# jaeyoungjo99/ELiMaLoc

Measured on AMD Instinct MI355X. Metric: ICP registrations/sec, 128k-pt scan vs 10M-pt map; pose err vs CPU ref, higher is better.
Workload: dtype f64

## Files before the change

### elimaloc_amd/_lib.py

```python
import ctypes as C
import os

_HERE = os.path.dirname(os.path.abspath(__file__))
LIB_PATH = os.environ.get("ELM_LIB") or os.path.join(_HERE, "libelimaloc_hip.so")

ELM_OK = 0
P2P, GICP, VGICP, AVGICP = 0, 1, 2, 3
MAX_ITER_TRACE = 64
PACKED_SUMS = 32
COMM_ID_BYTES = 128


class ElmError(RuntimeError):
    pass


class RegConfig(C.Structure):
    _fields_ = [
        ("i_max_thread", C.c_int32),
        ("icp_method", C.c_int32),
        ("voxel_search_method", C.c_int32),
        ("use_radar_cov", C.c_int32),
        ("max_iteration", C.c_int32),
        ("b_debug_print", C.c_int32),
# ... 109 lines not shown
                ("max_score_points", C.c_int32), ("top_k", C.c_int32), ("nms_xy_m", C.c_double), ("nms_yaw_deg", C.c_double),
                ("pool_min", C.c_int32), ("max_kz_span", C.c_int32), ("bitmap_max_bytes", C.c_int64)]


class GlobalRelocStats(C.Structure):
    _fields_ = [("lattice_poses", C.c_int64), ("valid_leaves", C.c_int64), ("nx", C.c_int32), ("ny", C.c_int32), ("n_yaw", C.c_int32),
                ("levels", C.c_int32), ("n_counted", C.c_int32), ("passes", C.c_int32), ("tau", C.c_uint32), ("_pad", C.c_uint32),
                ("nodes_bounded", C.c_int64 * 24), ("nodes_kept", C.c_int64 * 24), ("leaves_scored", C.c_int64), ("point_evals", C.c_int64),
                ("ms_ground", C.c_double), ("ms_search", C.c_double), ("ms_refine", C.c_double)]


ALLREDUCE_FN = C.CFUNCTYPE(C.c_int, C.c_void_p, C.c_size_t, C.c_void_p, C.c_void_p)

EXPORTS = [
    "elm_reg_config_default", "elm_ctx_create", "elm_ctx_create_multi", "elm_ctx_group_info", "elm_register_shard", "elm_ctx_destroy", "elm_last_error", "elm_strerror",
    "elm_ctx_synchronize", "elm_ctx_stream", "elm_ctx_set_profiling", "elm_ctx_set_work_counters", "elm_ctx_get_profile", "elm_map_build", "elm_map_destroy", "elm_map_cal_voxel_cov_all",
    "elm_map_cal_point_cov_all", "elm_map_build_neighbourhoods", "elm_map_get_info", "elm_map_empty", "elm_map_download_points",
    "elm_map_download_voxels", "elm_map_find_ground_height", "elm_map_get_correspondences", "elm_align_clouds_local", "elm_scan_upload", "elm_scan_destroy",
    "elm_scan_size", "elm_scan_download", "elm_register", "elm_format_register_log", "elm_register_batch", "elm_register_stream", "elm_register_stream_host", "elm_host_alloc", "elm_host_free", "elm_ctx_measure_h2d", "elm_register_batch_enqueue",
    "elm_register_batch_finish", "elm_deskew", "elm_deskew_downsample", "elm_deskew_prepare", "elm_comm_get_unique_id", "elm_comm_init",
    "elm_comm_destroy", "elm_comm_info", "elm_comm_set_hook", "elm_filter_points_by_distance", "elm_voxel_downsample",
    "elm_get_interpolated_pose", "elm_shape_odom_covariance", "elm_cal_frame_point_cov",
    "elm_ekf_config_default", "elm_ekf_create", "elm_ekf_destroy", "elm_ekf_predict_imu", "elm_ekf_predict", "elm_ekf_update_can", "elm_gps_project", "elm_ekf_update_navsatfix",
    "elm_ekf_update_pose", "elm_ekf_update_pcm_odom", "elm_ekf_get_state", "elm_ekf_publish",
    "elm_ini_load", "elm_ini_destroy", "elm_ini_get_string", "elm_ini_get_int", "elm_ini_get_bool", "elm_ini_get_double",
    "elm_ini_get_array", "elm_pcm_node_config_default", "elm_load_pcm_config", "elm_load_ekf_config", "elm_pcd_load_xyz",
    "elm_free", "elm_scan_from_cloud", "elm_pcm_callback_point_cloud",
    "elm_reloc_config_default", "elm_reloc_make_hypotheses", "elm_map_score_poses", "elm_relocalize",
    "elm_reloc_global_config_default", "elm_map_ground_heights", "elm_reloc_global_hypotheses", "elm_relocalize_global",
]

# ... 63 lines not shown
    L.elm_ctx_group_info.argtypes = [vp, C.POINTER(C.c_int), C.POINTER(C.c_int), C.POINTER(C.c_int), C.c_int]
    L.elm_register_shard.argtypes = [vp, vp, fp, C.c_size_t, C.c_size_t, dp, C.POINTER(RegConfig), C.POINTER(RegResult), C.POINTER(IterTrace), C.c_int]
    L.elm_ctx_destroy.restype = None
    L.elm_last_error.argtypes = [vp]
    L.elm_last_error.restype = C.c_char_p
    L.elm_strerror.argtypes = [C.c_int]
    L.elm_strerror.restype = C.c_char_p
    L.elm_ctx_synchronize.argtypes = [vp]
    L.elm_ctx_stream.argtypes = [vp]
    L.elm_ctx_stream.restype = vp
    L.elm_format_register_log.argtypes = [C.POINTER(RegConfig), C.POINTER(RegResult), C.c_size_t, C.POINTER(IterTrace), C.POINTER(C.c_double),
                                          C.c_double, C.c_char_p, C.c_size_t]
    L.elm_format_register_log.restype = C.c_size_t
    L.elm_ctx_set_profiling.argtypes = [vp, C.c_int]
    L.elm_ctx_set_work_counters.argtypes = [vp, C.c_int]
    L.elm_ctx_get_profile.argtypes = [vp, C.POINTER(Profile), C.c_int]
    L.elm_map_build.argtypes = [vp, fp, C.c_size_t, C.c_double, C.c_int, C.POINTER(vp)]
    L.elm_map_destroy.argtypes = [vp]
    L.elm_map_destroy.restype = None
    L.elm_map_cal_voxel_cov_all.argtypes = [vp]
    L.elm_map_cal_point_cov_all.argtypes = [vp, C.c_double]
    L.elm_map_build_neighbourhoods.argtypes = [vp]
    L.elm_map_get_info.argtypes = [vp, C.POINTER(MapInfo)]
    L.elm_map_empty.argtypes = [vp]
    L.elm_map_download_points.argtypes = [vp, dp, dp, dp, C.c_size_t]
    L.elm_map_download_voxels.argtypes = [vp, C.POINTER(C.c_int32), C.POINTER(C.c_int32), dp, dp, C.c_size_t]
    L.elm_map_find_ground_height.argtypes = [vp, C.c_double, C.c_double, dp, ip]
    L.elm_cal_frame_point_cov.argtypes = [dp, C.c_size_t, C.c_double, C.c_double, C.c_double, dp]
    L.elm_align_clouds_local.argtypes = [vp, C.c_int, dp, dp, dp, dp, C.c_size_t, dp, C.c_double, C.POINTER(RegConfig), dp, dp, dp]
    L.elm_map_get_correspondences.argtypes = [vp, vp, C.c_int, dp, C.c_size_t, C.c_double, C.POINTER(C.c_uint32), C.POINTER(C.c_int32), C.c_size_t, C.POINTER(C.c_size_t)]
# ... 95 lines not shown
```

### elimaloc_amd/csrc/elm_api.cpp

```cpp
#include <dlfcn.h>
#include <hip/hip_runtime.h>
#include <math.h>
#include <stdio.h>
#include <stdlib.h>
#include <string.h>
#include <unistd.h>

#include <algorithm>
#include <chrono>
#include <map>
#include <mutex>
#include <new>
#include <set>
#include <string>
#include <thread>
#include <vector>

#include "elm_hostapi.hpp"
#include "elm_internal.hpp"
#include "elm_la.hpp"

using namespace elm;

struct DevBuf {
// ... 62 lines not shown
    int device = 0;
    uint64_t id = 0;
    hipStream_t stream = nullptr;
    hipStream_t copy_stream = nullptr, order_stream = nullptr, poll_stream = nullptr;
    hipEvent_t ev_iter[4] = {nullptr, nullptr, nullptr, nullptr};
    std::vector<hipEvent_t> ev_groups;
    uint16_t* d_hilbert = nullptr;
    DevBuf d_order_jobs, d_order_tmp, d_arena, d_raw, d_flagged, d_asym;
    DevBuf d_q0, d_q1, d_q2, d_q3, d_q4, d_q5;
    DevBuf d_reloc[16];
    bool work_counters = false;
    void* h_jobs = nullptr;
    size_t h_jobs_cap = 0;
    std::string last_error;
    DevBuf d_scans, d_state, d_partials, d_sums, d_T0, d_trace, d_stage_pts, d_active, d_queue, d_ds;
    int stream_hint_count = 0, stream_hint_slots = 0, stream_hint_iters = 0;
    int* h_active = nullptr;
    int iter_hint = 0;
    int iter_ring[8] = {0, 0, 0, 0, 0, 0, 0, 0};
    unsigned iter_ring_pos = 0;
    const void* iter_key_map = nullptr;
    int iter_key_method = -1, iter_key_batch = 0;
    void* h_state = nullptr;
    size_t h_state_cap = 0;
    void* h_trace = nullptr;
    size_t h_trace_cap = 0;
    void* h_stage = nullptr;
    size_t h_stage_cap = 0;
    std::vector<uint32_t> h_key, h_ord, h_tmp;
    std::vector<struct elm_scan*> scan_free;
// ... 170 lines not shown
    {
        std::lock_guard<std::mutex> lk(g_live_mu);
        if (!g_live_ctx.erase(ctx)) return;
    }
    (void)hipSetDevice(ctx->device);
    if (ctx->stream) (void)hipStreamSynchronize(ctx->stream);
    if (ctx->comm && g_rccl.comm_destroy) g_rccl.comm_destroy(ctx->comm);
    for (hipStream_t st : {ctx->copy_stream, ctx->order_stream, ctx->poll_stream})
        if (st) { (void)hipStreamSynchronize(st); (void)hipStreamDestroy(st); }
    for (hipEvent_t e : {ctx->ev_iter[0], ctx->ev_iter[1], ctx->ev_iter[2], ctx->ev_iter[3]})
        if (e) (void)hipEventDestroy(e);
    for (hipEvent_t e : ctx->ev_groups) (void)hipEventDestroy(e);
    if (ctx->d_hilbert) (void)hipFree(ctx->d_hilbert);
    if (ctx->h_jobs) (void)hipHostFree(ctx->h_jobs);
    DevBuf* bufs[] = {&ctx->d_scans, &ctx->d_state, &ctx->d_partials, &ctx->d_sums, &ctx->d_T0, &ctx->d_trace, &ctx->d_stage_pts, &ctx->d_active, &ctx->d_queue, &ctx->d_ds,
                      &ctx->d_order_jobs, &ctx->d_order_tmp, &ctx->d_arena, &ctx->d_raw, &ctx->d_flagged, &ctx->d_asym, &ctx->d_q0, &ctx->d_q1, &ctx->d_q2, &ctx->d_q3, &ctx->d_q4, &ctx->d_q5};
    if (ctx->h_active) (void)hipHostFree(ctx->h_active);
    for (DevBuf* b : bufs)
        if (b->p) (void)hipFree(b->p);
    for (DevBuf& b : ctx->d_reloc)
        if (b.p) (void)hipFree(b.p);
    for (auto& b : ctx->scan_pool) (void)hipFree(b.first);
    for (elm_scan* f : ctx->scan_free) delete f;
    if (ctx->h_state) (void)hipHostFree(ctx->h_state);
    if (ctx->h_trace) (void)hipHostFree(ctx->h_trace);
    if (ctx->h_stage) (void)hipHostFree(ctx->h_stage);
    if (ctx->h_desc) (void)hipHostFree(ctx->h_desc);
    for (hipEvent_t e : ctx->events) (void)hipEventDestroy(e);
    if (ctx->stream) (void)hipStreamDestroy(ctx->stream);
    delete ctx;
}

extern "C" const char* elm_last_error(const elm_ctx* ctx) { return ctx ? ctx->last_error.c_str() : ""; }
extern "C" void* elm_ctx_stream(elm_ctx* ctx) { return ctx ? (void*)ctx->stream : nullptr; }
extern "C" int elm_ctx_set_work_counters(elm_ctx* ctx, int enable) {
    if (!ctx) return ELM_ERR_INVALID;
    if (ctx->in_flight) return ELM_ERR_INVALID;
    if (group_call(ctx)) return elm_multi::set_work_counters(ctx, enable);
    ctx->work_counters = enable != 0;
    return ELM_OK;
}

extern "C" int elm_ctx_set_profiling(elm_ctx* ctx, int enable) {
    if (!ctx) return ELM_ERR_INVALID;
    ctx->profiling = enable != 0;
    return ELM_OK;
}
extern "C" int elm_ctx_get_profile(elm_ctx* ctx, elm_profile* out, int reset) {
    if (!ctx || !out) return ELM_ERR_INVALID;
// ... 1578 lines not shown
    rp.method = cfg->icp_method;
    rp.max_iter = cfg->max_iteration;
    rp.uniform_blocks = uniform_blocks;
    rp.radar = pc.radar ? (cfg->use_radar_cov != 0 ? 1 : 2) : 0;
    rp.stats = ctx->work_counters ? 1 : 0;
    rp.radar_var[0] = cfg->range_variance_m;
    rp.radar_var[1] = cfg->azimuth_variance_deg;
    rp.radar_var[2] = cfg->elevation_variance_deg;
    if (pc.asym) {
        int rc;
        if ((rc = dev_reserve(ctx, ctx->d_asym, (size_t)std::max<uint32_t>(blocks, 1) * kAsymRecord * sizeof(double))) != ELM_OK) return rc;
        rp.asym = (double*)ctx->d_asym.p;
        rp.asym_sums = (double*)ctx->d_sums.p + (size_t)n_scans * kSums;
    }
    rp.rank_check = ((ctx->comm || ctx->hook) && !rp.radar && !rp.stats) ? 1 : 0;
    ctx->rp = rp;
    return ELM_OK;
}

static bool reg_args_ok(const elm_ctx* ctx, const elm_map* map, const elm_reg_config* cfg) {
    return map->ctx == ctx && cfg->icp_method >= ELM_P2P && cfg->icp_method <= ELM_AVGICP && !ctx->in_flight;
}

struct StateTail {
    int32_t active;
    int32_t rank_mismatch;
    int32_t _pad0[2];
    uint32_t ds_kept;
    int32_t ds_overflow;
    int32_t _pad1[10];
// ... 1074 lines not shown
```

### elimaloc_amd/csrc/elm_internal.hpp

```cpp
#pragma once
#include <hip/hip_runtime.h>
#include <stdint.h>

#include "../../include/elimaloc_hip.h"

namespace elm {

struct __attribute__((aligned(32))) HashSlot {
    int32_t kx, ky, kz;
    int32_t vid;
    uint32_t start;
    uint32_t cnt;
    uint32_t pad0, pad1;
};

struct __attribute__((packed, aligned(4))) Pt3 {
    float x, y, z;
};

struct __attribute__((aligned(16))) GridBlk {
    float x[4], y[4], z[4];
};

struct __attribute__((aligned(64))) VoxRec {
// ... 84 lines not shown

struct ScanState {
    double T[16];
    double Rinv[9];
    double tinv[3];
    double fitness;
    double local_cov[36];
    double n_corr_last;
    double pt_iters, cand_total, occ_total, fallback_blocks, tested_total;
    int32_t done;
    int32_t success;
    int32_t gate;
    int32_t iters;
    int32_t reg;
    int32_t _pad;
};

struct QueueItem {
    const Pt3* pts;
    uint32_t n, n_total;
};
struct StreamCtrl {
    int32_t next;
    int32_t completed;
    int32_t total;
    int32_t ready;
    int32_t done_iter;
};

struct StreamArgs {
// ... 17 lines not shown
    double max_fitness;
    int32_t method;
    int32_t max_iter;
    uint32_t uniform_blocks;
    int32_t radar;
    int32_t _reserved0;
    int32_t stats;
    uint32_t* flagged;
    int32_t rank_check;
    int32_t _pad_rc;
    double* asym;
    double* asym_sums;
    double radar_var[3];
    const double* query;
    int32_t* q_out;
};
constexpr int kAsymRecord = 16;
constexpr int kRadarRecord = 64;

constexpr int kTileShift = 3, kTile = 1 << kTileShift;
constexpr int kBlock = 256;
constexpr int kInitPack = 8;
struct InitPack {
    ScanDesc d[kInitPack];
    double T0[kInitPack][16];
};
constexpr int kSums = ELM_PACKED_SUMS;

void launch_init_state(hipStream_t s, ScanState* st, const double* T0, int batch, int map_empty, int* active);
void launch_init_pack(hipStream_t s, ScanDesc* scans, ScanState* st, const InitPack& pack, int batch, int map_empty, int* active, const unsigned* n_dev);
void launch_stream_refill(hipStream_t s, ScanDesc* scans, ScanState* st, int slots, const QueueItem* queue, const double* qT0,
                          ScanState* out_state, StreamCtrl* ctrl, int first, int save = 1);
// ... 108 lines not shown
```

### elimaloc_amd/csrc/elm_k_grid.hip

```cpp
#include <float.h>
#include <algorithm>
#include <hip/hip_runtime.h>

#include "elm_internal.hpp"
#include "elm_la.hpp"
#include "elm_dev_grid.hpp"

namespace elm {

template <int METHOD, int COMPACT, int TILED, int STATS, int WIDE>
__global__ __launch_bounds__(kBlock, (METHOD == ELM_P2P ? (STATS ? 7 : kGridWaves) : kGicpWaves)) void k_accumulate_grid(
       const DevMap m, const ScanDesc* __restrict__ scans, int batch,
                                                                            unsigned total_blocks, const ScanState* __restrict__ st,
                                                                            double* __restrict__ partials, const RegParams rp) {
    constexpr int kStats = (STATS == 1) ? 1 : 0;
    constexpr bool QUERY = STATS == 2;
    constexpr int NV = (METHOD == ELM_P2P) ? (kStats ? kP2PVals : kP2PVals - 3) : kSums;
    __shared__ double s_buf[kRedPass * kBlock];
    __shared__ double s_red[kSums];
    __shared__ int s_res[kBlock];
    __shared__ int s_tst[kStats ? kBlock : 1];
    __shared__ float s_pz[METHOD == ELM_P2P ? kBlock : 1];
    __shared__ unsigned s_st[kStats ? kBlock : 1];
    __shared__ unsigned s_cnt[kBlock / 64];
// ... 21 lines not shown
        double* p = s_buf + threadIdx.x;
        p[4 * kBlock] = a; p[5 * kBlock] = b; p[6 * kBlock] = c; p[7 * kBlock] = d;
    };
    auto load_g = [&](double& gx, double& gy, double& gz, float& pxf, float& pyf) {
        const double* p = s_buf + threadIdx.x;
        gx = p[4 * kBlock]; gy = p[5 * kBlock]; gz = p[6 * kBlock];
        const double w = p[7 * kBlock];
        pxf = __int_as_float(__double2loint(w)); pyf = __int_as_float(__double2hiint(w));
    };
    auto transform = [&](const float4 pf, double& px, double& py, double& pz, double& gx, double& gy, double& gz) {
        px = pf.x; py = pf.y; pz = pf.z;
        gx = ((S.T[0] * px + S.T[4] * py) + S.T[8] * pz) + S.T[12];
        gy = ((S.T[1] * px + S.T[5] * py) + S.T[9] * pz) + S.T[13];
        gz = ((S.T[2] * px + S.T[6] * py) + S.T[10] * pz) + S.T[14];
    };
    if (valid) {
        double px, py, pz, gx, gy, gz;
        float4 pf = make_float4(0.f, 0.f, 0.f, 0.f);
        if (QUERY) {
            gx = rp.query[3 * (size_t)i]; gy = rp.query[3 * (size_t)i + 1]; gz = rp.query[3 * (size_t)i + 2];
            px = py = pz = 0.0;
        } else {
            const Pt3 p3 = sd.pts[i];
            pf = make_float4(p3.x, p3.y, p3.z, 0.f);
            transform(pf, px, py, pz, gx, gy, gz);
        }
        const GridAxis ax = grid_axis(gx, m), ay = grid_axis(gy, m), az = grid_axis(gz, m);
        unsigned stat = 0;
        if (kStats && !TILED) {
            const int ux = ax.f - m.vx0, uy = ay.f - m.vy0, uz = az.f - m.vz0;
            const bool in_box = (unsigned)ux < (unsigned)m.vnx && (unsigned)uy < (unsigned)m.vny && (unsigned)uz < (unsigned)m.vnz;
            const unsigned sidx = in_box ? ((unsigned)ux * (unsigned)m.vny + (unsigned)uy) * (unsigned)m.vnz + (unsigned)uz : 0u;
            stat = m.vox_stat[sidx];
            stat = in_box ? stat : 0u;
        }
        float rho_u = 3e38f;
        int bx0, bx1, by0, by1, bz0, bz1;
        int ox, oy, oz;
        float dxo, dyo, dzo;
        grid_lean(ax, bx0, bx1, rho_u, ox, dxo);
        grid_lean(ay, by0, by1, rho_u, oy, dyo);
        grid_lean(az, bz0, bz1, rho_u, oz, dzo);
        (void)oz; (void)dzo;
        const int rx0 = bx0 - m.gx0, rx1 = bx1 - m.gx0, ry0 = by0 - m.gy0, ry1 = by1 - m.gy0, rz0 = bz0 - m.gz0, rz1 = bz1 - m.gz0;
        const bool inside = rx0 >= 0 && rx1 < m.gnx && rx0 <= rx1 && ry0 >= 0 && ry1 < m.gny && ry0 <= ry1 && rz0 >= 0 && rz1 < m.gnz && rz0 <= rz1;
        unsigned sb[4];
        int cb[5];
        cb[0] = 0;
        const float ex_ = fmaxf(dxo * (float)h - 1e-6f, 0.f), ey_ = fmaxf(dyo * (float)h - 1e-6f, 0.f);
        const float Bx = fminf(ex_ * ex_, 1e36f), By = fminf(ey_ * ey_, 1e36f);
        const bool xfirst = Bx <= By, has_x = rx1 != rx0, has_y = ry1 != ry0;
        unsigned s0[4], s1[4], s2[4];
        bool ok[4];
        ok[0] = inside;
        ok[1] = inside && (xfirst ? has_x : has_y);
        ok[2] = inside && (xfirst ? has_y : has_x);
        ok[3] = inside && has_x && has_y;
        if (!TILED) {
            const int own_x = ox ? rx1 : rx0, own_y = oy ? ry1 : ry0;
            const unsigned base = ((unsigned)own_x * (unsigned)m.gny + (unsigned)own_y) * (unsigned)m.gnz + (unsigned)rz0;
            const unsigned xs = (unsigned)m.gny * (unsigned)m.gnz, ys = (unsigned)m.gnz;
            const unsigned cx_n = ox ? base - xs : base + xs, cy_n = oy ? base - ys : base + ys, cd = ox ? cy_n - xs : cy_n + xs;
            unsigned cellv[4];
            cellv[0] = base; cellv[1] = xfirst ? cx_n : cy_n; cellv[2] = xfirst ? cy_n : cx_n; cellv[3] = cd;
#pragma unroll
            for (int k = 0; k < 4; ++k) {
                const uint32_t* e = m.grid_start + (ok[k] ? cellv[k] : 0u);
                s0[k] = e[0]; s1[k] = e[1]; s2[k] = e[2];
            }
        } else {
            const int own_x = ox ? rx1 : rx0, oth_x = ox ? rx0 : rx1, own_y = oy ? ry1 : ry0, oth_y = oy ? ry0 : ry1;
            int cxv[4], cyv[4];
            cxv[0] = own_x; cyv[0] = own_y;
            cxv[1] = xfirst ? oth_x : own_x; cyv[1] = xfirst ? own_y : oth_y;
            cxv[2] = xfirst ? own_x : oth_x; cyv[2] = xfirst ? oth_y : own_y;
            cxv[3] = oth_x; cyv[3] = oth_y;
#pragma unroll
            for (int k = 0; k < 4; ++k) {
                int zc0, nzc;
                const uint32_t* e = col_cells<1>(m, ok[k] ? cxv[k] : 0, ok[k] ? cyv[k] : 0, rz0, rz1, zc0, nzc);
                s0[k] = e[0]; s1[k] = e[nzc]; s2[k] = s1[k];
            }
        }
        float rr = (rho_u < 1e30f) ? (rho_u * (float)h - 1.1e-6f) * 0.999998f : 1e18f;
        float rr2 = (rr > 0.f) ? rr * rr * 0.999999f : -1.f;
        float ghx = (float)gx, ghy = (float)gy, ghz = (float)gz;
        const float eg = (fabsf(ghx) + fabsf(ghy) + fabsf(ghz)) * 5.9604652e-08f;
        float egrr = (2.0f * eg * fmaxf(rr, 0.f) + eg * eg) * 1.000001f;
        float egblk = (7.0f * eg * (float)h + eg * eg) * 1.000001f;
        float L1 = fminf(Bx, By), L2 = fmaxf(Bx, By), L3 = (Bx + By) * 0.999999f;
        asm volatile("" : "+v"(rr2), "+v"(ghx), "+v"(ghy), "+v"(ghz), "+v"(egrr), "+v"(egblk), "+v"(L1), "+v"(L2), "+v"(L3));
        stash_w(gx, gy, gz, __hiloint2double(__float_as_int(pf.y), __float_as_int(pf.x)));
        if (METHOD == ELM_P2P) s_pz[threadIdx.x] = pf.z;
        if (kStats) s_st[threadIdx.x] = stat;
        {
            int b0v[4], b1v[4];
#pragma unroll
            for (int k = 0; k < 4; ++k) {
                b0v[k] = ok[k] ? (int)s0[k] : 0;
                b1v[k] = ok[k] ? (int)((rz1 > rz0 || TILED) ? s2[k] : s1[k]) : 0;
            }
#pragma unroll
            for (int k = 0; k < 4; ++k) {
                sb[k] = (unsigned)(b0v[k] - cb[k]) * kBlkStep;
                cb[k + 1] = cb[k] + (b1v[k] - b0v[k]);
            }
        }
        {
            int nblk = cb[4];
            const f32x2 gxy = {ghx, ghy}, gzz = {ghz, 0.f};
            unsigned m1 = 0x7F800000u, m2 = 0x7F800000u;
            unsigned jb = 0;
            for (int t0 = 0; t0 < nblk; t0 += kBlocksPerTrip) {
                unsigned pb[kBlocksPerTrip];
#pragma unroll
                for (int w = 0; w < kBlocksPerTrip; ++w) {
                    const int t = t0 + w;
                    unsigned b_ = sb[3];
#pragma unroll
                    for (int k = 2; k >= 0; --k) b_ = (t < cb[k + 1]) ? sb[k] : b_;
                    pb[w] = (t < nblk) ? b_ + (unsigned)t * kBlkStep : 0u;
                }
                GridBlk B[kBlocksPerTrip];
#pragma unroll
                for (int w = 0; w < kBlocksPerTrip; ++w)
                    B[w] = *reinterpret_cast<const GridBlk*>(reinterpret_cast<const char*>(lp) + (WIDE ? ((size_t)pb[w] << 4) : (size_t)pb[w]));
                __builtin_amdgcn_sched_barrier(0);
#pragma unroll
                for (int w = 0; w < kBlocksPerTrip; ++w) {
                    f32x2 da, db;
                    blk_dist_h(B[w], gxy, gzz, da, db);
                    const unsigned was = m1;
                    two_smallest(da.x, 0u, m1, m2);
                    two_smallest(da.y, 1u, m1, m2);
                    two_smallest(db.x, 2u, m1, m2);
                    two_smallest(db.y, 3u, m1, m2);
                    jb = (m1 != was) ? pb[w] : jb;
                }
                const float dbest = __uint_as_float(m1 & ~3u);
                const float best = (dbest < rr2) ? (dbest + dbest * 7.62939453125e-06f + 2.0f * egrr) * 1.000001f : __builtin_inff();
                nblk = (L1 > best) ? cb[1] : ((L2 > best) ? cb[2] : ((L3 > best) ? cb[3] : nblk));
            }
            n_tested = 4 * nblk;
            hard = true;
            if (jb > 0) {
                const float d1 = __uint_as_float(m1 & ~3u), d2 = __uint_as_float(m2 & ~3u);
                const float r2 = d1 + d1 * 3.814697265625e-06f + egrr;
                hr2 = d1 + d1 * 3.814697265625e-06f + egblk;
                if (d2 - d2 * 3.814697265625e-06f > r2 + egrr && r2 < rr2) {
                    bj = (int)(jb / kBlkStep) * 4 + (int)(m1 & 3u);
                    hard = false;
                }
            }
        }
    }
    const unsigned long long hm = __ballot(hard);
    const unsigned lane = threadIdx.x & 63u, wave = threadIdx.x >> 6;
    if (lane == 0) s_cnt[wave] = (unsigned)__popcll(hm);
    __syncthreads();
    unsigned n_hard = 0, my_slot = 0;
#pragma unroll
    for (unsigned w = 0; w < kBlock / 64; ++w) {
        my_slot += (w < wave) ? s_cnt[w] : 0u;
        n_hard += s_cnt[w];
    }
    my_slot += (unsigned)__popcll(hm & ((1ull << lane) - 1ull));
    if (n_hard) {
        GridHardRec* __restrict__ s_rec = reinterpret_cast<GridHardRec*>(s_buf);
        if (hard) {
// ... 13 lines not shown
            const GridHardRec R = s_rec[live ? it : 0];
            int win, walked;
            grid_ball_walk<TILED, LPI>(m, lp, R, live, rl, lane, win, walked);
            if (kStats) walked = group_sum_int<LPI>(walked);
            if (rl == 0 && live) {
                s_res[it] = win;
                if (kStats) s_tst[it] = walked;
            }
        }
        __syncthreads();
        if (hard) {
            bj = s_res[my_slot];
            if (kStats) n_tested += s_tst[my_slot];
        }
        __syncthreads();
    }
    if (QUERY) {
        if (valid) {
            double gx, gy, gz;
            float pxf, pyf;
            load_g(gx, gy, gz, pxf, pyf);
            int out = -2;
            if (bj >= 0) {
                const Pt3 q = blk_point(lp, bj);
                const double ex = (double)q.x - gx, ey = (double)q.y - gy, ez = (double)q.z - gz;
                if ((ex * ex + ey * ey) + ez * ez < rp.th2) out = (int)m.grid_idx[bj];
            } else if ((gx * gx + gy * gy) + gz * gz < rp.th2) {
                out = -1;
            }
            rp.q_out[i] = out;
// ... 127 lines not shown
```

### elimaloc_amd/csrc/elm_k_solve.hip

```cpp
#include <float.h>
#include <algorithm>
#include <hip/hip_runtime.h>

#include "elm_internal.hpp"
#include "elm_la.hpp"
#include "elm_dev_reduce.hpp"

namespace elm {

__device__ void update_inverse(ScanState& S) {
    double R[9];
    for (int r = 0; r < 3; ++r)
        for (int c = 0; c < 3; ++c) R[r * 3 + c] = S.T[c * 4 + r];
    inv3(R, S.Rinv);
    for (int r = 0; r < 3; ++r)
        S.tinv[r] = -((S.Rinv[r * 3] * S.T[12] + S.Rinv[r * 3 + 1] * S.T[13]) + S.Rinv[r * 3 + 2] * S.T[14]);
}

__device__ void init_scan_state(ScanState& S, const double* __restrict__ T0, int reg, int map_empty) {
    for (int k = 0; k < 16; ++k) S.T[k] = T0[k];
    update_inverse(S);
    S.fitness = 0.0;
    for (int k = 0; k < 36; ++k) S.local_cov[k] = (k % 7 == 0) ? 1.0 : 0.0;
    S.n_corr_last = 0.0;
    S.pt_iters = 0.0; S.cand_total = 0.0; S.occ_total = 0.0; S.fallback_blocks = 0.0; S.tested_total = 0.0;
    S.done = map_empty ? 1 : 0;
    S.success = 0;
    S.gate = map_empty ? 1 : 0;
    S.iters = 0;
    S.reg = reg;
    S._pad = 0;
}

__global__ __launch_bounds__(64) void k_init_state(ScanState* st, const double* __restrict__ T0, int batch, int map_empty,
                                                   int* active) {
    const int s = blockIdx.x * 64 + threadIdx.x;
    if (s >= batch) return;
    if (!map_empty) atomicAdd(active, 1);
    init_scan_state(st[s], T0 + (size_t)s * 16, s, map_empty);
}

__global__ __launch_bounds__(64) void k_init_pack(ScanDesc* scans, ScanState* st, const InitPack pack, int batch, int map_empty, int* active,
                                                  const unsigned* __restrict__ n_dev) {
    const int s = threadIdx.x;
    if (s == 0) { active[0] = map_empty ? 0 : batch; active[1] = 0; }
    if (s >= batch) return;
// ... 258 lines not shown
            const QueueItem q = sa.queue[r];
            sa.scans[s].pts = q.pts;
            sa.scans[s].n = q.n;
            sa.scans[s].n_total = q.n_total;
            for (int k = 0; k < 16; ++k) S.T[k] = T0[k];
            update_inverse(S);
            S.fitness = 0.0;
            S.n_corr_last = 0.0;
            S.pt_iters = 0.0; S.cand_total = 0.0; S.occ_total = 0.0; S.fallback_blocks = 0.0; S.tested_total = 0.0;
            S.done = 0;
            S.success = 0;
            S.gate = 0;
            S.iters = 0;
            S.reg = r;
            S._pad = 0;
        }
    } else if (lane == 0) {
        S.done = 1;
        S.reg = -1;
    }
}
__device__ __forceinline__ void finish_slot(const StreamArgs& sa, ScanState& S, int s) {
#if !defined(__gfx950__) && !defined(__gfx942__) && !defined(__gfx90a__) && defined(__HIP_DEVICE_COMPILE__)
#error "finish_slot relies on gfx9 memory ordering (one vmcnt for loads and stores, write-through vector L1)"
#endif
    constexpr int W = (int)(sizeof(ScanState) / sizeof(double));
    const int lane = threadIdx.x & 63;
    __builtin_amdgcn_fence(__ATOMIC_RELEASE, "workgroup");
    __builtin_amdgcn_s_waitcnt(0);
    __builtin_amdgcn_wave_barrier();
// ... 241 lines not shown
    rotvec_to_matrix(&x[3], dR);
    double Tn[16];
    for (int r = 0; r < 3; ++r) {
        for (int c = 0; c < 3; ++c)
            Tn[c * 4 + r] = (S.T[0 * 4 + r] * dR[0 * 3 + c] + S.T[1 * 4 + r] * dR[1 * 3 + c]) + S.T[2 * 4 + r] * dR[2 * 3 + c];
        Tn[12 + r] = ((S.T[0 * 4 + r] * x[0] + S.T[1 * 4 + r] * x[1]) + S.T[2 * 4 + r] * x[2]) + S.T[12 + r];
    }
    Tn[3] = 0.0; Tn[7] = 0.0; Tn[11] = 0.0; Tn[15] = 1.0;
    const double step = matrix_to_angle(dR) + sqrt((x[0] * x[0] + x[1] * x[1]) + x[2] * x[2]);
    if (tr && t < 36) tr->JTJ[t] = full36 ? full[lj * 6 + li] : hij;
    bool fin = false;
    if (lead) {
        S.fitness = fitness;
        for (int k = 0; k < 16; ++k) S.T[k] = Tn[k];
        update_inverse(S);
        if (tr) {
            for (int k = 0; k < 6; ++k) { tr->JTr[k] = tot[21 + k]; tr->x[k] = x[k]; }
            tr->residual_sum = tot[27];
            tr->n_corr = n_corr;
            tr->step_norm = step;
            for (int k = 0; k < 16; ++k) tr->T[k] = Tn[k];
        }
        if (step < rp.term_thr || iter >= rp.max_iter) {
            S.done = 1;
            atomicSub(active, 1);
            const bool bad = fitness > rp.max_fitness;
            S.success = bad ? 0 : 1;
            S.gate = bad ? 3 : 0;
            fin = true;
        }
// ... 151 lines not shown
```

### include/elimaloc_hip.h

```cpp
#ifndef ELIMALOC_HIP_H
#define ELIMALOC_HIP_H

#include <stddef.h>
#include <stdint.h>

#ifdef __cplusplus
extern "C" {
#endif

#define ELM_OK 0
#define ELM_ERR_INVALID -1
#define ELM_ERR_DEVICE -2
#define ELM_ERR_NO_DEVICE -3
#define ELM_ERR_COMM -4
#define ELM_ERR_UNSUPPORTED -5
#define ELM_ERR_IO -6
#define ELM_ERR_ALLOC -7

#define ELM_MAX_ITER_TRACE 64

typedef struct elm_ctx elm_ctx;
typedef struct elm_map elm_map;
typedef struct elm_scan elm_scan;

// ... 79 lines not shown
int elm_ctx_create(int device_id, elm_ctx** out);
void elm_ctx_destroy(elm_ctx* ctx);
const char* elm_last_error(const elm_ctx* ctx);
const char* elm_strerror(int status);
int elm_ctx_synchronize(elm_ctx* ctx);
void* elm_ctx_stream(elm_ctx* ctx);

typedef struct elm_profile {
    uint64_t accumulate_launches;
    uint64_t solve_steps;
    double accumulate_ms;
    double solve_ms;
} elm_profile;
int elm_ctx_set_profiling(elm_ctx* ctx, int enable);
int elm_ctx_set_work_counters(elm_ctx* ctx, int enable);
int elm_ctx_get_profile(elm_ctx* ctx, elm_profile* out, int reset);

int elm_map_build(elm_ctx* ctx, const float* xyz, size_t n, double voxel_size, int max_points_per_voxel,
                  elm_map** out);
void elm_map_destroy(elm_map* map);
int elm_map_cal_voxel_cov_all(elm_map* map);
int elm_map_cal_point_cov_all(elm_map* map, double d_search_dist);
int elm_map_build_neighbourhoods(elm_map* map);
int elm_map_get_info(const elm_map* map, elm_map_info* info);
int elm_map_empty(const elm_map* map);
int elm_map_download_points(const elm_map* map, double* xyz, double* cov9, double* mean3, size_t cap);
int elm_map_download_voxels(const elm_map* map, int32_t* key3, int32_t* npts, double* cov9, double* mean3,
                            size_t cap);
int elm_map_get_correspondences(elm_ctx* ctx, const elm_map* map, int what, const double* xyz, size_t n, double max_dist,
                                uint32_t* src_index, int32_t* tgt_index, size_t cap, size_t* n_pairs);
// ... 219 lines not shown
```

Measured before the change: 98320.

## Reuse certified nearest-neighbour results across ICP iterations via per-point safety radius

Stores, for each scan point, its nearest-neighbour index and a certified safety margin derived from the gap between the best and second-best distances and the voxel face distance. On later iterations a point keeps its old correspondence without re-searching when the pose update (rotation times point norm plus translation) stays below the remaining margin. Points that still need a search are compacted within the block so the grid search runs on fewer lanes. The path is gated behind a check_mode("reuse") / "reuse_verify" flag and adds shared-memory shuffles, syncthreads and a per-point certificate buffer.

```diff
diff --git a/elimaloc_amd/_lib.py b/elimaloc_amd/_lib.py
--- a/elimaloc_amd/_lib.py
+++ b/elimaloc_amd/_lib.py
@@ -147,7 +147,7 @@
 
 EXPORTS = [
     "elm_reg_config_default", "elm_ctx_create", "elm_ctx_create_multi", "elm_ctx_group_info", "elm_register_shard", "elm_ctx_destroy", "elm_last_error", "elm_strerror",
-    "elm_ctx_synchronize", "elm_ctx_stream", "elm_ctx_set_profiling", "elm_ctx_set_work_counters", "elm_ctx_get_profile", "elm_map_build", "elm_map_destroy", "elm_map_cal_voxel_cov_all",
+    "elm_ctx_synchronize", "elm_ctx_stream", "elm_ctx_set_profiling", "elm_ctx_set_work_counters", "elm_ctx_reuse_counters", "elm_ctx_get_profile", "elm_map_build", "elm_map_destroy", "elm_map_cal_voxel_cov_all",
     "elm_map_cal_point_cov_all", "elm_map_build_neighbourhoods", "elm_map_get_info", "elm_map_empty", "elm_map_download_points",
     "elm_map_download_voxels", "elm_map_find_ground_height", "elm_map_get_correspondences", "elm_align_clouds_local", "elm_scan_upload", "elm_scan_destroy",
     "elm_scan_size", "elm_scan_download", "elm_register", "elm_format_register_log", "elm_register_batch", "elm_register_stream", "elm_register_stream_host", "elm_host_alloc", "elm_host_free", "elm_ctx_measure_h2d", "elm_register_batch_enqueue",
@@ -241,6 +241,7 @@
     L.elm_format_register_log.restype = C.c_size_t
     L.elm_ctx_set_profiling.argtypes = [vp, C.c_int]
     L.elm_ctx_set_work_counters.argtypes = [vp, C.c_int]
+    L.elm_ctx_reuse_counters.argtypes = [vp, C.c_void_p]
     L.elm_ctx_get_profile.argtypes = [vp, C.POINTER(Profile), C.c_int]
     L.elm_map_build.argtypes = [vp, fp, C.c_size_t, C.c_double, C.c_int, C.POINTER(vp)]
     L.elm_map_destroy.argtypes = [vp]
diff --git a/elimaloc_amd/csrc/elm_api.cpp b/elimaloc_amd/csrc/elm_api.cpp
--- a/elimaloc_amd/csrc/elm_api.cpp
+++ b/elimaloc_amd/csrc/elm_api.cpp
@@ -100,6 +100,7 @@
     size_t h_jobs_cap = 0;
     std::string last_error;
     DevBuf d_scans, d_state, d_partials, d_sums, d_T0, d_trace, d_stage_pts, d_active, d_queue, d_ds;
+    DevBuf d_cert, d_reuse_cnt;
     int stream_hint_count = 0, stream_hint_slots = 0, stream_hint_iters = 0;
     int* h_active = nullptr;
     int iter_hint = 0;
@@ -300,7 +301,8 @@
     if (ctx->d_hilbert) (void)hipFree(ctx->d_hilbert);
     if (ctx->h_jobs) (void)hipHostFree(ctx->h_jobs);
     DevBuf* bufs[] = {&ctx->d_scans, &ctx->d_state, &ctx->d_partials, &ctx->d_sums, &ctx->d_T0, &ctx->d_trace, &ctx->d_stage_pts, &ctx->d_active, &ctx->d_queue, &ctx->d_ds,
-                      &ctx->d_order_jobs, &ctx->d_order_tmp, &ctx->d_arena, &ctx->d_raw, &ctx->d_flagged, &ctx->d_asym, &ctx->d_q0, &ctx->d_q1, &ctx->d_q2, &ctx->d_q3, &ctx->d_q4, &ctx->d_q5};
+                      &ctx->d_order_jobs, &ctx->d_order_tmp, &ctx->d_arena, &ctx->d_raw, &ctx->d_flagged, &ctx->d_asym, &ctx->d_q0, &ctx->d_q1, &ctx->d_q2, &ctx->d_q3, &ctx->d_q4, &ctx->d_q5,
+                      &ctx->d_cert, &ctx->d_reuse_cnt};
     if (ctx->h_active) (void)hipHostFree(ctx->h_active);
     for (DevBuf* b : bufs)
         if (b->p) (void)hipFree(b->p);
@@ -319,6 +321,14 @@
 
 extern "C" const char* elm_last_error(const elm_ctx* ctx) { return ctx ? ctx->last_error.c_str() : ""; }
 extern "C" void* elm_ctx_stream(elm_ctx* ctx) { return ctx ? (void*)ctx->stream : nullptr; }
+extern "C" int elm_ctx_reuse_counters(elm_ctx* ctx, unsigned long long* out) {
+    if (!ctx || !out) return ELM_ERR_INVALID;
+    HIPCHK(ctx, hipSetDevice(ctx->device));
+    HIPCHK(ctx, hipStreamSynchronize(ctx->stream));
+    memset(out, 0, kReuseCounters * sizeof(unsigned long long));
+    if (ctx->rp.reuse_cnt) HIPCHK(ctx, hipMemcpy(out, ctx->rp.reuse_cnt, kReuseCounters * sizeof(unsigned long long), hipMemcpyDeviceToHost));
+    return ELM_OK;
+}
 extern "C" int elm_ctx_set_work_counters(elm_ctx* ctx, int enable) {
     if (!ctx) return ELM_ERR_INVALID;
     if (ctx->in_flight) return ELM_ERR_INVALID;
@@ -1927,6 +1937,17 @@
         rp.asym_sums = (double*)ctx->d_sums.p + (size_t)n_scans * kSums;
     }
     rp.rank_check = ((ctx->comm || ctx->hook) && !rp.radar && !rp.stats) ? 1 : 0;
+    const bool reuse_verify = check_mode("reuse_verify");
+    if (pc.use_grid && !rp.radar && !rp.stats && (rp.method == ELM_P2P || rp.method == ELM_GICP) && (reuse_verify || check_mode("reuse"))) {
+        int rc;
+        if ((rc = dev_reserve(ctx, ctx->d_cert, (size_t)std::max<uint32_t>(blocks, 1) * kBlock * sizeof(uint2))) != ELM_OK) return rc;
+        rp.cert = (uint2*)ctx->d_cert.p;
+        if (reuse_verify) {
+            if ((rc = dev_reserve(ctx, ctx->d_reuse_cnt, kReuseCounters * sizeof(unsigned long long))) != ELM_OK) return rc;
+            HIPCHK(ctx, hipMemsetAsync(ctx->d_reuse_cnt.p, 0, kReuseCounters * sizeof(unsigned long long), ctx->stream));
+            rp.reuse_cnt = (unsigned long long*)ctx->d_reuse_cnt.p;
+        }
+    }
     ctx->rp = rp;
     return ELM_OK;
 }
diff --git a/elimaloc_amd/csrc/elm_internal.hpp b/elimaloc_amd/csrc/elm_internal.hpp
--- a/elimaloc_amd/csrc/elm_internal.hpp
+++ b/elimaloc_amd/csrc/elm_internal.hpp
@@ -122,6 +122,7 @@
     int32_t iters;
     int32_t reg;
     int32_t _pad;
+    double move_rot, move_t;
 };
 
 struct QueueItem {
@@ -169,8 +170,11 @@
     double radar_var[3];
     const double* query;
     int32_t* q_out;
+    uint2* cert;
+    unsigned long long* reuse_cnt;
 };
 constexpr int kAsymRecord = 16;
+constexpr int kReuseCounters = 64;
 constexpr int kRadarRecord = 64;
 
 constexpr int kTileShift = 3, kTile = 1 << kTileShift;
diff --git a/elimaloc_amd/csrc/elm_k_grid.hip b/elimaloc_amd/csrc/elm_k_grid.hip
--- a/elimaloc_amd/csrc/elm_k_grid.hip
+++ b/elimaloc_amd/csrc/elm_k_grid.hip
@@ -1,5 +1,6 @@
 #include <float.h>
 #include <algorithm>
+#include <type_traits>
 #include <hip/hip_runtime.h>
 
 #include "elm_internal.hpp"
@@ -59,8 +60,15 @@
         gy = ((S.T[1] * px + S.T[5] * py) + S.T[9] * pz) + S.T[13];
         gz = ((S.T[2] * px + S.T[6] * py) + S.T[10] * pz) + S.T[14];
     };
+    constexpr bool kReuse = STATS == 0;
+    uint2* __restrict__ cert = kReuse ? rp.cert : nullptr;
+    const bool warm = kReuse && cert != nullptr && S.iters > 0;
+    const bool verify = kReuse && rp.reuse_cnt != nullptr;
+    const size_t ci = (size_t)L * kBlock + threadIdx.x;
+    double gx = 0.0, gy = 0.0, gz = 0.0;
+    bool need = false, certd = false;
     if (valid) {
-        double px, py, pz, gx, gy, gz;
+        double px, py, pz;
         float4 pf = make_float4(0.f, 0.f, 0.f, 0.f);
         if (QUERY) {
             gx = rp.query[3 * (size_t)i]; gy = rp.query[3 * (size_t)i + 1]; gz = rp.query[3 * (size_t)i + 2];
@@ -70,134 +78,209 @@
             pf = make_float4(p3.x, p3.y, p3.z, 0.f);
             transform(pf, px, py, pz, gx, gy, gz);
         }
-        const GridAxis ax = grid_axis(gx, m), ay = grid_axis(gy, m), az = grid_axis(gz, m);
-        unsigned stat = 0;
-        if (kStats && !TILED) {
-            const int ux = ax.f - m.vx0, uy = ay.f - m.vy0, uz = az.f - m.vz0;
-            const bool in_box = (unsigned)ux < (unsigned)m.vnx && (unsigned)uy < (unsigned)m.vny && (unsigned)uz < (unsigned)m.vnz;
-            const unsigned sidx = in_box ? ((unsigned)ux * (unsigned)m.vny + (unsigned)uy) * (unsigned)m.vnz + (unsigned)uz : 0u;
-            stat = m.vox_stat[sidx];
-            stat = in_box ? stat : 0u;
-        }
-        float rho_u = 3e38f;
-        int bx0, bx1, by0, by1, bz0, bz1;
-        int ox, oy, oz;
-        float dxo, dyo, dzo;
-        grid_lean(ax, bx0, bx1, rho_u, ox, dxo);
-        grid_lean(ay, by0, by1, rho_u, oy, dyo);
-        grid_lean(az, bz0, bz1, rho_u, oz, dzo);
-        (void)oz; (void)dzo;
-        const int rx0 = bx0 - m.gx0, rx1 = bx1 - m.gx0, ry0 = by0 - m.gy0, ry1 = by1 - m.gy0, rz0 = bz0 - m.gz0, rz1 = bz1 - m.gz0;
-        const bool inside = rx0 >= 0 && rx1 < m.gnx && rx0 <= rx1 && ry0 >= 0 && ry1 < m.gny && ry0 <= ry1 && rz0 >= 0 && rz1 < m.gnz && rz0 <= rz1;
-        unsigned sb[4];
-        int cb[5];
-        cb[0] = 0;
-        const float ex_ = fmaxf(dxo * (float)h - 1e-6f, 0.f), ey_ = fmaxf(dyo * (float)h - 1e-6f, 0.f);
-        const float Bx = fminf(ex_ * ex_, 1e36f), By = fminf(ey_ * ey_, 1e36f);
-        const bool xfirst = Bx <= By, has_x = rx1 != rx0, has_y = ry1 != ry0;
-        unsigned s0[4], s1[4], s2[4];
-        bool ok[4];
-        ok[0] = inside;
-        ok[1] = inside && (xfirst ? has_x : has_y);
-        ok[2] = inside && (xfirst ? has_y : has_x);
-        ok[3] = inside && has_x && has_y;
-        if (!TILED) {
-            const int own_x = ox ? rx1 : rx0, own_y = oy ? ry1 : ry0;
-            const unsigned base = ((unsigned)own_x * (unsigned)m.gny + (unsigned)own_y) * (unsigned)m.gnz + (unsigned)rz0;
-            const unsigned xs = (unsigned)m.gny * (unsigned)m.gnz, ys = (unsigned)m.gnz;
-            const unsigned cx_n = ox ? base - xs : base + xs, cy_n = oy ? base - ys : base + ys, cd = ox ? cy_n - xs : cy_n + xs;
-            unsigned cellv[4];
-            cellv[0] = base; cellv[1] = xfirst ? cx_n : cy_n; cellv[2] = xfirst ? cy_n : cx_n; cellv[3] = cd;
-#pragma unroll
-            for (int k = 0; k < 4; ++k) {
-                const uint32_t* e = m.grid_start + (ok[k] ? cellv[k] : 0u);
-                s0[k] = e[0]; s1[k] = e[1]; s2[k] = e[2];
-            }
-        } else {
-            const int own_x = ox ? rx1 : rx0, oth_x = ox ? rx0 : rx1, own_y = oy ? ry1 : ry0, oth_y = oy ? ry0 : ry1;
-            int cxv[4], cyv[4];
-            cxv[0] = own_x; cyv[0] = own_y;
-            cxv[1] = xfirst ? oth_x : own_x; cyv[1] = xfirst ? own_y : oth_y;
-            cxv[2] = xfirst ? own_x : oth_x; cyv[2] = xfirst ? oth_y : own_y;
-            cxv[3] = oth_x; cyv[3] = oth_y;
-#pragma unroll
-            for (int k = 0; k < 4; ++k) {
-                int zc0, nzc;
-                const uint32_t* e = col_cells<1>(m, ok[k] ? cxv[k] : 0, ok[k] ? cyv[k] : 0, rz0, rz1, zc0, nzc);
-                s0[k] = e[0]; s1[k] = e[nzc]; s2[k] = s1[k];
-            }
-        }
-        float rr = (rho_u < 1e30f) ? (rho_u * (float)h - 1.1e-6f) * 0.999998f : 1e18f;
-        float rr2 = (rr > 0.f) ? rr * rr * 0.999999f : -1.f;
-        float ghx = (float)gx, ghy = (float)gy, ghz = (float)gz;
-        const float eg = (fabsf(ghx) + fabsf(ghy) + fabsf(ghz)) * 5.9604652e-08f;
-        float egrr = (2.0f * eg * fmaxf(rr, 0.f) + eg * eg) * 1.000001f;
-        float egblk = (7.0f * eg * (float)h + eg * eg) * 1.000001f;
-        float L1 = fminf(Bx, By), L2 = fmaxf(Bx, By), L3 = (Bx + By) * 0.999999f;
-        asm volatile("" : "+v"(rr2), "+v"(ghx), "+v"(ghy), "+v"(ghz), "+v"(egrr), "+v"(egblk), "+v"(L1), "+v"(L2), "+v"(L3));
         stash_w(gx, gy, gz, __hiloint2double(__float_as_int(pf.y), __float_as_int(pf.x)));
         if (METHOD == ELM_P2P) s_pz[threadIdx.x] = pf.z;
-        if (kStats) s_st[threadIdx.x] = stat;
-        {
-            int b0v[4], b1v[4];
-#pragma unroll
-            for (int k = 0; k < 4; ++k) {
-                b0v[k] = ok[k] ? (int)s0[k] : 0;
-                b1v[k] = ok[k] ? (int)((rz1 > rz0 || TILED) ? s2[k] : s1[k]) : 0;
-            }
-#pragma unroll
-            for (int k = 0; k < 4; ++k) {
-                sb[k] = (unsigned)(b0v[k] - cb[k]) * kBlkStep;
-                cb[k + 1] = cb[k] + (b1v[k] - b0v[k]);
-            }
-        }
-        {
-            int nblk = cb[4];
-            const f32x2 gxy = {ghx, ghy}, gzz = {ghz, 0.f};
-            unsigned m1 = 0x7F800000u, m2 = 0x7F800000u;
-            unsigned jb = 0;
-            for (int t0 = 0; t0 < nblk; t0 += kBlocksPerTrip) {
-                unsigned pb[kBlocksPerTrip];
-#pragma unroll
-                for (int w = 0; w < kBlocksPerTrip; ++w) {
-                    const int t = t0 + w;
-                    unsigned b_ = sb[3];
-#pragma unroll
-                    for (int k = 2; k >= 0; --k) b_ = (t < cb[k + 1]) ? sb[k] : b_;
-                    pb[w] = (t < nblk) ? b_ + (unsigned)t * kBlkStep : 0u;
-                }
-                GridBlk B[kBlocksPerTrip];
-#pragma unroll
-                for (int w = 0; w < kBlocksPerTrip; ++w)
-                    B[w] = *reinterpret_cast<const GridBlk*>(reinterpret_cast<const char*>(lp) + (WIDE ? ((size_t)pb[w] << 4) : (size_t)pb[w]));
-                __builtin_amdgcn_sched_barrier(0);
-#pragma unroll
-                for (int w = 0; w < kBlocksPerTrip; ++w) {
-                    f32x2 da, db;
-                    blk_dist_h(B[w], gxy, gzz, da, db);
-                    const unsigned was = m1;
-                    two_smallest(da.x, 0u, m1, m2);
-                    two_smallest(da.y, 1u, m1, m2);
-                    two_smallest(db.x, 2u, m1, m2);
-                    two_smallest(db.y, 3u, m1, m2);
-                    jb = (m1 != was) ? pb[w] : jb;
-                }
-                const float dbest = __uint_as_float(m1 & ~3u);
-                const float best = (dbest < rr2) ? (dbest + dbest * 7.62939453125e-06f + 2.0f * egrr) * 1.000001f : __builtin_inff();
-                nblk = (L1 > best) ? cb[1] : ((L2 > best) ? cb[2] : ((L3 > best) ? cb[3] : nblk));
-            }
-            n_tested = 4 * nblk;
-            hard = true;
-            if (jb > 0) {
-                const float d1 = __uint_as_float(m1 & ~3u), d2 = __uint_as_float(m2 & ~3u);
-                const float r2 = d1 + d1 * 3.814697265625e-06f + egrr;
-                hr2 = d1 + d1 * 3.814697265625e-06f + egblk;
-                if (d2 - d2 * 3.814697265625e-06f > r2 + egrr && r2 < rr2) {
-                    bj = (int)(jb / kBlkStep) * 4 + (int)(m1 & 3u);
-                    hard = false;
-                }
-            }
-        }
+        need = true;
+        if (warm) {
+            const uint2 rec = cert[ci];
+            const float sr = __uint_as_float(rec.y);
+            const float pn = __builtin_sqrtf((pf.x * pf.x + pf.y * pf.y) + pf.z * pf.z);
+            const float g1 = (float)(fabs(gx) + fabs(gy) + fabs(gz));
+            const float dl = fmaf((float)S.move_rot, pn, (float)S.move_t) * 1.00001f + fmaf(1e-12f, g1, 1e-9f);
+            certd = dl < sr;
+            if (certd) {
+                bj = (int)rec.x;
+                cert[ci] = make_uint2(rec.x, __float_as_uint((sr - dl) * 0.99999905f));
+            }
+            need = !certd || verify;
+            if (verify) {
+                const unsigned it = (unsigned)min(S.iters, 15);
+                const unsigned long long el = __ballot(sr > 0.f), ce = __ballot(certd), al = __ballot(true);
+                if ((threadIdx.x & 63u) == (unsigned)(__ffsll((long long)al) - 1)) {
+                    atomicAdd(&rp.reuse_cnt[it * 4 + 0], (unsigned long long)__popcll(el));
+                    atomicAdd(&rp.reuse_cnt[it * 4 + 1], (unsigned long long)__popcll(ce));
+                    atomicAdd(&rp.reuse_cnt[it * 4 + 3], (unsigned long long)__popcll(al));
+                }
+            }
+        }
+    }
+    bool active = valid;
+    unsigned owner = threadIdx.x;
+    if (warm) {
+        const unsigned long long nm = __ballot(need);
+        const unsigned qlane = threadIdx.x & 63u, qwave = threadIdx.x >> 6;
+        if (qlane == 0) s_cnt[qwave] = (unsigned)__popcll(nm);
+        s_buf[threadIdx.x] = __hiloint2double(__float_as_int(__builtin_inff()), bj);
+        s_buf[kBlock + threadIdx.x] = __hiloint2double(0, 0);
+        __syncthreads();
+        unsigned n_need = 0, my_q = 0;
+#pragma unroll
+        for (unsigned w = 0; w < kBlock / 64; ++w) {
+            my_q += (w < qwave) ? s_cnt[w] : 0u;
+            n_need += s_cnt[w];
+        }
+        my_q += (unsigned)__popcll(nm & ((1ull << qlane) - 1ull));
+        if (need) s_res[my_q] = (int)threadIdx.x;
+        __syncthreads();
+        active = threadIdx.x < n_need;
+        if (active) {
+            owner = (unsigned)s_res[threadIdx.x];
+            const double* q = s_buf + owner;
+            gx = q[4 * kBlock]; gy = q[5 * kBlock]; gz = q[6 * kBlock];
+        }
+    }
+    float cs = -1.f;
+    if (active) {
+            const GridAxis ax = grid_axis(gx, m), ay = grid_axis(gy, m), az = grid_axis(gz, m);
+            unsigned stat = 0;
+            if (kStats && !TILED) {
+                const int ux = ax.f - m.vx0, uy = ay.f - m.vy0, uz = az.f - m.vz0;
+                const bool in_box = (unsigned)ux < (unsigned)m.vnx && (unsigned)uy < (unsigned)m.vny && (unsigned)uz < (unsigned)m.vnz;
+                const unsigned sidx = in_box ? ((unsigned)ux * (unsigned)m.vny + (unsigned)uy) * (unsigned)m.vnz + (unsigned)uz : 0u;
+                stat = m.vox_stat[sidx];
+                stat = in_box ? stat : 0u;
+            }
+            float vface = 0.f;
+            if (kReuse) {
+                const float ux = (float)(ax.cg & 1) + ax.fr, uy = (float)(ay.cg & 1) + ay.fr, uz = (float)(az.cg & 1) + az.fr;
+                vface = fminf(fminf(fminf(ux, 2.f - ux), fminf(uy, 2.f - uy)), fminf(uz, 2.f - uz)) * (float)h;
+            }
+            float rho_u = 3e38f;
+            int bx0, bx1, by0, by1, bz0, bz1;
+            int ox, oy, oz;
+            float dxo, dyo, dzo;
+            grid_lean(ax, bx0, bx1, rho_u, ox, dxo);
+            grid_lean(ay, by0, by1, rho_u, oy, dyo);
+            grid_lean(az, bz0, bz1, rho_u, oz, dzo);
+            (void)oz; (void)dzo;
+            const int rx0 = bx0 - m.gx0, rx1 = bx1 - m.gx0, ry0 = by0 - m.gy0, ry1 = by1 - m.gy0, rz0 = bz0 - m.gz0, rz1 = bz1 - m.gz0;
+            const bool inside = rx0 >= 0 && rx1 < m.gnx && rx0 <= rx1 && ry0 >= 0 && ry1 < m.gny && ry0 <= ry1 && rz0 >= 0 && rz1 < m.gnz && rz0 <= rz1;
+            unsigned sb[4];
+            int cb[5];
+            cb[0] = 0;
+            const float ex_ = fmaxf(dxo * (float)h - 1e-6f, 0.f), ey_ = fmaxf(dyo * (float)h - 1e-6f, 0.f);
+            const float Bx = fminf(ex_ * ex_, 1e36f), By = fminf(ey_ * ey_, 1e36f);
+            const bool xfirst = Bx <= By, has_x = rx1 != rx0, has_y = ry1 != ry0;
+            unsigned s0[4], s1[4], s2[4];
+            bool ok[4];
+            ok[0] = inside;
+            ok[1] = inside && (xfirst ? has_x : has_y);
+            ok[2] = inside && (xfirst ? has_y : has_x);
+            ok[3] = inside && has_x && has_y;
+            if (!TILED) {
+                const int own_x = ox ? rx1 : rx0, own_y = oy ? ry1 : ry0;
+                const unsigned base = ((unsigned)own_x * (unsigned)m.gny + (unsigned)own_y) * (unsigned)m.gnz + (unsigned)rz0;
+                const unsigned xs = (unsigned)m.gny * (unsigned)m.gnz, ys = (unsigned)m.gnz;
+                const unsigned cx_n = ox ? base - xs : base + xs, cy_n = oy ? base - ys : base + ys, cd = ox ? cy_n - xs : cy_n + xs;
+                unsigned cellv[4];
+                cellv[0] = base; cellv[1] = xfirst ? cx_n : cy_n; cellv[2] = xfirst ? cy_n : cx_n; cellv[3] = cd;
+    #pragma unroll
+                for (int k = 0; k < 4; ++k) {
+                    const uint32_t* e = m.grid_start + (ok[k] ? cellv[k] : 0u);
+                    s0[k] = e[0]; s1[k] = e[1]; s2[k] = e[2];
+                }
+            } else {
+                const int own_x = ox ? rx1 : rx0, oth_x = ox ? rx0 : rx1, own_y = oy ? ry1 : ry0, oth_y = oy ? ry0 : ry1;
+                int cxv[4], cyv[4];
+                cxv[0] = own_x; cyv[0] = own_y;
+                cxv[1] = xfirst ? oth_x : own_x; cyv[1] = xfirst ? own_y : oth_y;
+                cxv[2] = xfirst ? own_x : oth_x; cyv[2] = xfirst ? oth_y : own_y;
+                cxv[3] = oth_x; cyv[3] = oth_y;
+    #pragma unroll
+                for (int k = 0; k < 4; ++k) {
+                    int zc0, nzc;
+                    const uint32_t* e = col_cells<1>(m, ok[k] ? cxv[k] : 0, ok[k] ? cyv[k] : 0, rz0, rz1, zc0, nzc);
+                    s0[k] = e[0]; s1[k] = e[nzc]; s2[k] = s1[k];
+                }
+            }
+            float rr = (rho_u < 1e30f) ? (rho_u * (float)h - 1.1e-6f) * 0.999998f : 1e18f;
+            float rr2 = (rr > 0.f) ? rr * rr * 0.999999f : -1.f;
+            float ghx = (float)gx, ghy = (float)gy, ghz = (float)gz;
+            const float eg = (fabsf(ghx) + fabsf(ghy) + fabsf(ghz)) * 5.9604652e-08f;
+            float egrr = (2.0f * eg * fmaxf(rr, 0.f) + eg * eg) * 1.000001f;
+            float egblk = (7.0f * eg * (float)h + eg * eg) * 1.000001f;
+            float L1 = fminf(Bx, By), L2 = fmaxf(Bx, By), L3 = (Bx + By) * 0.999999f;
+            asm volatile("" : "+v"(rr2), "+v"(ghx), "+v"(ghy), "+v"(ghz), "+v"(egrr), "+v"(egblk), "+v"(L1), "+v"(L2), "+v"(L3));
+            if (kStats) s_st[threadIdx.x] = stat;
+            {
+                int b0v[4], b1v[4];
+    #pragma unroll
+                for (int k = 0; k < 4; ++k) {
+                    b0v[k] = ok[k] ? (int)s0[k] : 0;
+                    b1v[k] = ok[k] ? (int)((rz1 > rz0 || TILED) ? s2[k] : s1[k]) : 0;
+                }
+    #pragma unroll
+                for (int k = 0; k < 4; ++k) {
+                    sb[k] = (unsigned)(b0v[k] - cb[k]) * kBlkStep;
+                    cb[k + 1] = cb[k] + (b1v[k] - b0v[k]);
+                }
+            }
+            {
+                int nblk = cb[4];
+                const f32x2 gxy = {ghx, ghy}, gzz = {ghz, 0.f};
+                unsigned m1 = 0x7F800000u, m2 = 0x7F800000u;
+                unsigned jb = 0;
+                for (int t0 = 0; t0 < nblk; t0 += kBlocksPerTrip) {
+                    unsigned pb[kBlocksPerTrip];
+    #pragma unroll
+                    for (int w = 0; w < kBlocksPerTrip; ++w) {
+                        const int t = t0 + w;
+                        unsigned b_ = sb[3];
+    #pragma unroll
+                        for (int k = 2; k >= 0; --k) b_ = (t < cb[k + 1]) ? sb[k] : b_;
+                        pb[w] = (t < nblk) ? b_ + (unsigned)t * kBlkStep : 0u;
+                    }
+                    GridBlk B[kBlocksPerTrip];
+    #pragma unroll
+                    for (int w = 0; w < kBlocksPerTrip; ++w)
+                        B[w] = *reinterpret_cast<const GridBlk*>(reinterpret_cast<const char*>(lp) + (WIDE ? ((size_t)pb[w] << 4) : (size_t)pb[w]));
+                    __builtin_amdgcn_sched_barrier(0);
+    #pragma unroll
+                    for (int w = 0; w < kBlocksPerTrip; ++w) {
+                        f32x2 da, db;
+                        blk_dist_h(B[w], gxy, gzz, da, db);
+                        const unsigned was = m1;
+                        two_smallest(da.x, 0u, m1, m2);
+                        two_smallest(da.y, 1u, m1, m2);
+                        two_smallest(db.x, 2u, m1, m2);
+                        two_smallest(db.y, 3u, m1, m2);
+                        jb = (m1 != was) ? pb[w] : jb;
+                    }
+                    const float dbest = __uint_as_float(m1 & ~3u);
+                    const float best = (dbest < rr2) ? (dbest + dbest * 7.62939453125e-06f + 2.0f * egrr) * 1.000001f : __builtin_inff();
+                    nblk = (L1 > best) ? cb[1] : ((L2 > best) ? cb[2] : ((L3 > best) ? cb[3] : nblk));
+                }
+                n_tested = 4 * nblk;
+                hard = true;
+                if (jb > 0) {
+                    const float d1 = __uint_as_float(m1 & ~3u), d2 = __uint_as_float(m2 & ~3u);
+                    const float r2 = d1 + d1 * 3.814697265625e-06f + egrr;
+                    hr2 = d1 + d1 * 3.814697265625e-06f + egblk;
+                    if (d2 - d2 * 3.814697265625e-06f > r2 + egrr && r2 < rr2) {
+                        bj = (int)(jb / kBlkStep) * 4 + (int)(m1 & 3u);
+                        hard = false;
+                        if (kReuse) {
+                            const float lcut = (nblk <= cb[1]) ? L1 : ((nblk <= cb[2]) ? fminf(L2, L3) : ((nblk <= cb[3]) ? L3 : __builtin_inff()));
+                            const float dlo = fmaxf(fminf(fminf(d2 - d2 * 3.814697265625e-06f, rr2) - egrr, lcut), 0.f);
+                            cs = fminf(0.5f * (__builtin_sqrtf(dlo) - __builtin_sqrtf(r2)), vface) * 0.9999847412109375f - 1e-6f;
+                        }
+                    }
+                }
+            }
+    }
+    if (warm) {
+        if (active) {
+            s_buf[owner] = __hiloint2double(__float_as_int(hr2), bj);
+            s_buf[kBlock + owner] = __hiloint2double(hard ? 1 : 0, __float_as_int(hard ? 0.f : cs));
+        }
+        __syncthreads();
+        const double a = s_buf[threadIdx.x], c = s_buf[kBlock + threadIdx.x];
+        bj = __double2loint(a);
+        hr2 = __int_as_float(__double2hiint(a));
+        hard = __double2hiint(c) != 0;
+        if (need && !certd) cert[ci] = make_uint2((unsigned)bj, (unsigned)__double2loint(c));
+    } else if (cert && valid) {
+        cert[ci] = make_uint2((unsigned)bj, __float_as_uint(hard ? 0.f : cs));
     }
     const unsigned long long hm = __ballot(hard);
     const unsigned lane = threadIdx.x & 63u, wave = threadIdx.x >> 6;
@@ -241,6 +324,15 @@
             if (kStats) n_tested += s_tst[my_slot];
         }
         __syncthreads();
+    }
+    if (warm && verify) {
+        bool bad = false;
+        if (valid) {
+            const uint2 rec = cert[ci];
+            bad = __uint_as_float(rec.y) > 0.f && (int)rec.x != bj;
+        }
+        const unsigned long long bm = __ballot(bad);
+        if ((threadIdx.x & 63u) == 0 && bm) atomicAdd(&rp.reuse_cnt[(unsigned)min(S.iters, 15) * 4 + 2], (unsigned long long)__popcll(bm));
     }
     if (QUERY) {
         if (valid) {
diff --git a/elimaloc_amd/csrc/elm_k_solve.hip b/elimaloc_amd/csrc/elm_k_solve.hip
--- a/elimaloc_amd/csrc/elm_k_solve.hip
+++ b/elimaloc_amd/csrc/elm_k_solve.hip
@@ -30,6 +30,7 @@
     S.iters = 0;
     S.reg = reg;
     S._pad = 0;
+    S.move_rot = __builtin_inf(); S.move_t = __builtin_inf();
 }
 
 __global__ __launch_bounds__(64) void k_init_state(ScanState* st, const double* __restrict__ T0, int batch, int map_empty,
@@ -318,6 +319,7 @@
             S.iters = 0;
             S.reg = r;
             S._pad = 0;
+            S.move_rot = __builtin_inf(); S.move_t = __builtin_inf();
         }
     } else if (lane == 0) {
         S.done = 1;
@@ -589,6 +591,9 @@
         S.fitness = fitness;
         for (int k = 0; k < 16; ++k) S.T[k] = Tn[k];
         update_inverse(S);
+        constexpr double kUp = 1.0 + 0x1p-40;
+        S.move_t = sqrt((x[0] * x[0] + x[1] * x[1]) + x[2] * x[2]) * kUp + 1e-12;
+        S.move_rot = sqrt((x[3] * x[3] + x[4] * x[4]) + x[5] * x[5]) * kUp + 1e-12;
         if (tr) {
             for (int k = 0; k < 6; ++k) { tr->JTr[k] = tot[21 + k]; tr->x[k] = x[k]; }
             tr->residual_sum = tot[27];
diff --git a/include/elimaloc_hip.h b/include/elimaloc_hip.h
--- a/include/elimaloc_hip.h
+++ b/include/elimaloc_hip.h
@@ -117,6 +117,7 @@
 } elm_profile;
 int elm_ctx_set_profiling(elm_ctx* ctx, int enable);
 int elm_ctx_set_work_counters(elm_ctx* ctx, int enable);
+int elm_ctx_reuse_counters(elm_ctx* ctx, unsigned long long* out);
 int elm_ctx_get_profile(elm_ctx* ctx, elm_profile* out, int reset);
 
 int elm_map_build(elm_ctx* ctx, const float* xyz, size_t n, double voxel_size, int max_points_per_voxel,
```

After: 90900, median of 2. 7.5% lower.
